# precice/fem-shell

Measured on AMD Instinct MI355X. Metric: elements assembled/s + CG iters/s, 4M-tri shell, 1/2/4/8 MI355X, higher is better.
Workload: dtype f64; 1 GPU; configs[3] flat panel 1414x1414 squares: 3998792 tri3, 12013350 dofs; parallelism=row-partition x1, rccl_ranks_seen=0, assembly_step=one femshell_assemble: launch + status round trip, warmup_step=one femshell_assemble + cg_iters CG iterations

## Files before the change

fem-shell_amd/binding.py:

```python
import ctypes as C
import os
import subprocess

import numpy as np

_HERE = os.path.dirname(os.path.abspath(__file__))
_CSRC = os.path.join(_HERE, "csrc")

REF_Y21 = 0x1
REF_DRILL_MAX = 0x2
REASSEMBLE_EACH_SOLVE = 0x4
REF_DEFAULT = REF_Y21 | REF_DRILL_MAX
REORDER_MORTON = 0x10
REORDER_RCM = 0x20

KERNEL_ASSEMBLE, KERNEL_SPMV, KERNEL_CG_UPDATE, KERNEL_CG_DIRECTION = 0, 1, 2, 3
KERNEL_LUMPED_MASS, KERNEL_MASS_SHIFT, KERNEL_NEWMARK_RHS, KERNEL_NEWMARK_UPDATE = 4, 5, 6, 7
KERNEL_SPMM, KERNEL_GRAM, KERNEL_BLOCK_COMBINE = 8, 9, 10
KERNEL_ELEMENT_PRODUCT = 11
KERNEL_ELEMENT_RESULTANTS = 12
KERNEL_ELEMENT_LOADS = 13
KERNEL_GEOMETRIC_PRODUCT = 14

SYMBOLS = [
    "femshell_create", "femshell_destroy", "femshell_last_error", "femshell_set_mesh",
    "femshell_set_dirichlet", "femshell_set_loads", "femshell_assemble", "femshell_assemble_async", "femshell_solve",
    "femshell_get_solution", "femshell_residual_history", "femshell_element_matrices",
    "femshell_nnz_blocks", "femshell_export_bsr", "femshell_spmv", "femshell_row_begin",
    "femshell_row_end", "femshell_comm_unique_id", "femshell_comm_init", "femshell_time_kernel",
    "femshell_sync", "femshell_pc_defaults", "femshell_set_preconditioner", "femshell_amg_levels", "femshell_amg_level",
    "femshell_amg_export", "femshell_residual", "femshell_comm_ranks", "femshell_amg_setup_stats", "femshell_amg_dense_stats", "femshell_amg_partition_info", "femshell_assembly_kernel",
    "femshell_amg_cycle_bytes", "femshell_comm_selftest", "femshell_comm_counters", "femshell_owned_nodes", "femshell_comm_bytes", "femshell_set_initial_guess",
    "femshell_amg_patch_info", "femshell_amg_symbolic_info", "femshell_pc_apply", "femshell_set_sections",
    "femshell_set_density", "femshell_lumped_mass", "femshell_dynamics_defaults", "femshell_dynamics_begin", "femshell_dynamics_step",
    "femshell_dynamics_accept", "femshell_dynamics_state", "femshell_dynamics_energy", "femshell_dynamics_end",
    "femshell_modal_defaults", "femshell_modes", "femshell_spmm", "femshell_modal_gram",
    "femshell_set_prescribed", "femshell_reactions", "femshell_element_product", "femshell_element_resultants",
    "femshell_set_element_loads", "femshell_element_load_vector",
    "femshell_geometric_product", "femshell_buckling_defaults", "femshell_buckling",
    "femshell_pool_stats", "femshell_amg_device_dense_inverse", "femshell_amg_dense_apply",
    "femshell_amg_device_block_jacobi", "femshell_block_jacobi_export", "femshell_block_jacobi_apply",
]


class FemShellError(RuntimeError):
    def __init__(self, code, msg):
# ... 123 lines not shown
    L.femshell_sync.argtypes = [vp]
    L.femshell_pc_defaults.argtypes = [C.c_int32, C.POINTER(PcOptions)]
    L.femshell_set_preconditioner.argtypes = [vp, C.POINTER(PcOptions)]
    L.femshell_amg_levels.argtypes = [vp]
    L.femshell_amg_levels.restype = C.c_int32
    L.femshell_amg_level.argtypes = [vp, C.c_int32, C.POINTER(AmgLevelInfo)]
    L.femshell_amg_export.argtypes = [vp, C.c_int32, C.c_int32, C.c_void_p]
    L.femshell_amg_export.restype = C.c_int64
    L.femshell_amg_setup_stats.argtypes = [vp, dp]
    L.femshell_amg_dense_stats.argtypes = [vp, dp]
    L.femshell_amg_patch_info.argtypes = [vp, dp]
    L.femshell_amg_symbolic_info.argtypes = [vp, ip]
    L.femshell_pc_apply.argtypes = [vp, dp, dp]
    L.femshell_amg_partition_info.argtypes = [vp, dp]
    L.femshell_assembly_kernel.argtypes = [vp]
    L.femshell_comm_selftest.argtypes = [vp, dp]
    L.femshell_comm_counters.argtypes = [vp, C.POINTER(C.c_int64), C.c_int32]
    L.femshell_comm_bytes.argtypes = [vp, C.POINTER(C.c_int64), C.c_int32]
    L.femshell_amg_cycle_bytes.argtypes = [vp, dp, C.c_int32]
    L.femshell_amg_cycle_bytes.restype = C.c_int32
    L.femshell_set_density.argtypes = [vp, C.c_double, C.c_int32, dp]
    L.femshell_lumped_mass.argtypes = [vp, dp]
    L.femshell_dynamics_defaults.argtypes = [C.POINTER(DynamicsOptions)]
    L.femshell_dynamics_begin.argtypes = [vp, C.POINTER(DynamicsOptions), dp, dp]
    L.femshell_dynamics_step.argtypes = [vp, C.c_double, C.c_int32, C.POINTER(SolveInfo)]
    L.femshell_dynamics_accept.argtypes = [vp]
    L.femshell_dynamics_state.argtypes = [vp, C.c_int32, dp, dp, dp]
    L.femshell_dynamics_energy.argtypes = [vp, C.c_int32, dp]
    L.femshell_dynamics_end.argtypes = [vp]
    L.femshell_modal_defaults.argtypes = [C.POINTER(ModalOptions)]
# ... 388 lines not shown
        _check(self._L.femshell_amg_setup_stats(self._h, _d(out)))
        return {"prolongator_ms": out[0], "ap_ms": out[1], "restriction_ms": out[2], "galerkin_ms": out[3],
                "galerkin_useful_flops": out[4], "galerkin_mfma_flops_issued": out[5], "galerkin_on_matrix_cores": bool(out[6])}

    def amg_symbolic_info(self):
        out = np.zeros(3, dtype=np.int32)
        _check(self._L.femshell_amg_symbolic_info(self._h, _i(out)))
        return {"in_hbm": int(out[0]), "host_after_overflow": int(out[1]), "host_by_rule": int(out[2])}

    def assembly_kernel(self):
        k = self._L.femshell_assembly_kernel(self._h)
        if k < 0:
            _check(k)
        return "k_assemble_pipe" if k == 1 else "k_assemble"

    def amg_dense_stats(self):
        out = np.zeros(6)
        _check(self._L.femshell_amg_dense_stats(self._h, _d(out)))
        return {"n": int(out[0]), "ms": out[1], "mfma_flops_issued": out[2], "useful_flops": out[3], "dropped_directions": int(out[4]),
                "bytes": out[5]}

    def amg_device_dense_inverse(self, rowptr, colidx, vals, single_precision=False):
        rowptr = np.ascontiguousarray(rowptr, dtype=np.int32)
        colidx = np.ascontiguousarray(colidx, dtype=np.int32)
        vals = np.ascontiguousarray(vals, dtype=np.float64)
        n = 6 * (len(rowptr) - 1)
        inv, out = np.zeros((n, n)), np.zeros(6)
        _check(self._L.femshell_amg_device_dense_inverse(self._h, len(rowptr) - 1, _i(rowptr), _i(colidx), _d(vals),
                                                         1 if single_precision else 0, _d(inv), _d(out)))
        return inv, {"n": int(out[0]), "ms": out[1], "mfma_flops_issued": out[2], "useful_flops": out[3],
# ... 370 lines not shown
```

fem-shell_amd/csrc/api.cpp:

```cpp
#include "api_internal.hpp"
#include "reorder.hpp"

#include <algorithm>
#include <atomic>
#include <chrono>
#include <cmath>
#include <cstdio>
#include <cstdlib>
#include <cstring>

using namespace femshell;

namespace femshell {

namespace {
thread_local std::string g_err;

struct ProductBuffers {
    DevBuf<double> x, y;
    std::vector<double> stage;
    int upload(femshell_ctx *c, NodeOrder order, const double *hx)
    {
        const size_t ld = (size_t)c->plan.n_local_nodes() * 6;
        FS_HIP(y.alloc((size_t)c->plan.n_pad * 6));
// ... 614 lines not shown
    if (!c || !out) return set_err(FEMSHELL_ERR_INVALID, "femshell_comm_bytes: null argument");
    out[0] = c->comm.halo_bytes_sent;
    out[1] = c->comm.collective_bytes;
    if (clear) c->comm.halo_bytes_sent = c->comm.collective_bytes = 0;
    return c->comm.active() ? 1 : 0;
}

int femshell_comm_selftest(femshell_ctx *c, double out_us[3])
{
    if (!c || !out_us) return set_err(FEMSHELL_ERR_INVALID, "femshell_comm_selftest: null argument");
    for (int i = 0; i < 3; i++) out_us[i] = c->comm_selftest_done ? c->comm_selftest_us[i] : -1.0;
    return c->comm_selftest_done ? 1 : 0;
}

int32_t femshell_comm_ranks(femshell_ctx *c) { return c ? comm_count(c->comm) : 0; }

static int set_mesh_on_this_rank(femshell_ctx *c, int32_t n_nodes, const double *xyz, int32_t n_tri, const int32_t *tri,
                                 int32_t n_quad, const int32_t *quad)
{
    int rc = FEMSHELL_OK;
    TraceRange trace("femshell_set_mesh (plan + upload)");
    static const bool verbose = plan_verbose();
    double t_part = wall_s();
    auto part_done = [&](const char *what) {
        const double t = wall_s();
        if (verbose) fprintf(stderr, "[femshell set_mesh] %-40s %.3f s\n", what, t - t_part);
        t_part = t;
    };
    if (!all_finite(xyz, 3ll * n_nodes)) return set_err(FEMSHELL_ERR_MESH, "femshell_set_mesh: non-finite coordinate");
    std::string e;
// ... 103 lines not shown
    c->dm.cols = c->cols.p;
    c->dm.pair_ptr = c->pair_ptr.p;
    c->dm.slice_elem_ptr = c->slice_elem_ptr.p;
    c->dm.slice_elem_nodes = reinterpret_cast<const int4 *>(c->slice_elem_nodes.p);
    c->dm.max_slice_elems = p.max_slice_elems;
    c->dm.max_slice_width = p.max_slice_width;
    c->dm.item_ptr = c->item_ptr.p;
    c->dm.slice_desc = reinterpret_cast<const int4 *>(c->slice_desc.p);
    c->dm.items = reinterpret_cast<const uint4 *>(c->items.p);
    FS_HIP(c->item_flags.alloc(p.pipe ? 0 : p.items.size()));
    c->dm.item_flags = c->item_flags.p;
    c->dm.max_stage_rows = p.max_stage_rows;
    c->dm.pipe = p.pipe ? 1 : 0;
    c->pipe_without_sections = p.pipe;
    c->dm.slice_elem_ptr_last = (int32_t)(p.slice_elem_nodes.size() / 4);
    {
        const size_t lds = assemble_lds_layout(c->dm, p.max_slice_elems, p.max_stage_rows, p.n_lquad() > 0);
        if (p.max_slice_width > 64) return set_err(FEMSHELL_ERR_UNSUPPORTED, "femshell_set_mesh: a node has more than 63 neighbours");
        if (lds > 160 * 1024)
            return set_err(FEMSHELL_ERR_UNSUPPORTED, "femshell_set_mesh: a 32-node slice touches too many elements for the LDS staging");
    }
    c->dm.vals = c->vals.p;
    c->dm.symmetric = p.symmetric ? 1 : 0;
    c->dm.diag_upper = (p.symmetric && knob_flag("FEMSHELL_DIAG_UPPER", true)) ? 1 : 0;
    c->dm.max_in_width = p.max_in_width;
    c->dm.in_width = c->in_width.p;
    c->dm.in_base = c->in_base.p;
    c->dm.in_slots = c->in_slots.p;
    c->dm.in_rows = c->in_rows.p;
    const bool local_products = p.symmetric && p.max_loc > 0 && knob_flag("FEMSHELL_SPMV_LOCAL", true);
// ... 123 lines not shown
static int upload_item_layout(femshell_ctx *c, bool sections)
{
    const Plan &p = c->plan;
    hipStream_t st = c->stream;
    FS_HIP(hipStreamSynchronize(st));
    FS_HIP(c->item_ptr.upload(p.item_ptr, st));
    FS_HIP(c->slice_desc.upload(p.slice_desc, st));
    FS_HIP(c->items.upload(p.items, st));
    FS_HIP(c->item_flags.alloc(p.pipe ? 0 : p.items.size()));
    c->dm.item_ptr = c->item_ptr.p;
    c->dm.slice_desc = reinterpret_cast<const int4 *>(c->slice_desc.p);
    c->dm.items = reinterpret_cast<const uint4 *>(c->items.p);
    c->dm.item_flags = c->item_flags.p;
    c->dm.max_stage_rows = p.max_stage_rows;
    c->dm.pipe = p.pipe ? 1 : 0;
    (void)assemble_lds_layout(c->dm, p.max_slice_elems, p.max_stage_rows, p.n_lquad() > 0, sections);
    launch_item_flags(c->dm, (int64_t)p.items.size(), st);
    FS_HIP(hipGetLastError());
    FS_HIP(hipStreamSynchronize(st));
    return FEMSHELL_OK;
}

int femshell_set_sections(femshell_ctx *c, int32_t n_sections, const femshell_section *sections, const int32_t *tri_section,
                          const int32_t *quad_section)
{
    if (!c) return set_err(FEMSHELL_ERR_INVALID, "femshell_set_sections: null context");
    if (const int prc = finish_pending_assembly(c)) return prc;
    if (!c->have_mesh) return set_err(FEMSHELL_ERR_INVALID, "femshell_set_sections: call femshell_set_mesh first");
    if (c->dyn.active) return set_err(FEMSHELL_ERR_INVALID, "femshell_set_sections: not while dynamics is active (femshell_dynamics_end first)");
    if (n_sections < 0) return set_err(FEMSHELL_ERR_INVALID, "femshell_set_sections: n_sections < 0");
// ... 276 lines not shown
    if (!c) return set_err(FEMSHELL_ERR_INVALID, "femshell_amg_cycle_bytes: null context");
    if (!c->amg || !c->amg->valid) return set_err(FEMSHELL_ERR_INVALID, "femshell_amg_cycle_bytes: no multigrid hierarchy");
    std::vector<double> b;
    (void)amg_cycle_bytes(c, &b);
    for (int32_t l = 0; per_level != nullptr && l < cap && l < (int32_t)b.size(); l++) per_level[l] = b[(size_t)l];
    return (int32_t)b.size();
}

int femshell_assembly_kernel(femshell_ctx *c)
{
    if (!c) return set_err(FEMSHELL_ERR_INVALID, "femshell_assembly_kernel: null context");
    if (!c->have_mesh) return set_err(FEMSHELL_ERR_INVALID, "femshell_assembly_kernel: no mesh");
    return c->dm.pipe ? 1 : 0;
}

int femshell_amg_dense_stats(femshell_ctx *c, double out[6])
{
    if (!c || !out) return set_err(FEMSHELL_ERR_INVALID, "femshell_amg_dense_stats: null argument");
    if (!c->amg || !c->amg->valid) return set_err(FEMSHELL_ERR_INVALID, "femshell_amg_dense_stats: no multigrid hierarchy");
    const AmgDenseStats &S = c->amg->dense;
    out[0] = (double)S.n;
    out[1] = S.ms;
    out[2] = S.mfma_flops;
    out[3] = S.useful_flops;
    out[4] = (double)S.dropped;
    out[5] = S.bytes;
    return FEMSHELL_OK;
}

int femshell_amg_device_dense_inverse(femshell_ctx *c, int32_t n_nodes, const int32_t *rowptr, const int32_t *colidx, const double *vals,
// ... 453 lines not shown
```

fem-shell_amd/csrc/assemble_kernel.hpp:

```cpp
#pragma once

#include "device_common.hpp"
#include "kernels.hpp"
#include "plan.hpp"

namespace femshell {

__device__ __forceinline__ void lds_barrier()
{
    asm volatile("s_waitcnt lgkmcnt(0)\n\ts_barrier" ::: "memory");
}

template <int kWavesPerSimd, int kAblate = 0, bool kHasQuads = false, bool kSections = false>
__global__ __launch_bounds__(256, kWavesPerSimd) void k_assemble(DeviceMatrix m, MatConst mc, DeviceSections ds)
{
    extern __shared__ double lds[];
    double *lds_rec = lds + m.lds_rec_off;
    double *lds_stage = lds + m.lds_stage_off;
    constexpr int kRec = kHasQuads ? kRecDoublesQuad : kRecDoubles;
    const int tid = threadIdx.x;
    constexpr int kThreads = 256;
    const int etid = kThreads - 1 - tid;

    unsigned long long tacc[8] = {0, 0, 0, 0, 0, 0, 0, 0}, tprev = 0;
// ... 334 lines not shown
    return __hiloint2double(hi2, lo2);
}

__device__ __forceinline__ double unspecified_double()
{
    double x;
    asm volatile("" : "=v"(x));
    return x;
}

constexpr int kPipeConsumers = 192;
constexpr int kPipeFlagShift = 9;
static_assert(kFlagDiagBit + 1 + kPipeFlagShift <= 32 && kFlagValenceMask >= (uint32_t)(kItemPairs * 255), "the constraint word must fit item.w and hold the count of 255 chunks");
constexpr int kPipeRecPasses = 3;

template <int kAblate = 0, bool kHasQuads = false, bool kSections = false>
__global__ __launch_bounds__(256, 2) void k_assemble_pipe(DeviceMatrix m, MatConst mc, DeviceSections ds)
{
    constexpr bool kSecConsume = kSections && !(kAblate & 256), kSecProduce = kSections && !(kAblate & 512);
    extern __shared__ double lds[];
    __shared__ int simd_of_wave[4];
    constexpr int kRec = kHasQuads ? kRecDoublesQuad : (kSections ? RecLeanSec::doubles : RecLean::doubles);
    constexpr int kCoords = kHasQuads ? 12 : 9;
    const int tid = threadIdx.x, lane = tid & 63, wave = tid >> 6;
    int vwave;
    {
        unsigned hw;
        asm volatile("s_getreg_b32 %0, hwreg(HW_REG_HW_ID)" : "=s"(hw));
        const int simd = (int)((hw >> 4) & 3u);
        if (lane == 0) simd_of_wave[wave] = simd;
        __syncthreads();
// ... 12 lines not shown
            asm volatile("s_memtime %0\n\ts_waitcnt lgkmcnt(0)" : "=s"(tnow)::"memory");
            if (slot >= 0) tacc[slot] += tnow - tprev;
            tprev = tnow;
        }
    };
    stamp(-1);
    auto desc_a_of = [&](int s_) { return (s_ < w.last) ? m.slice_desc[2 * s_] : make_int4(0, 0, 0, 0); };
    auto desc_b_of = [&](int s_) { return (s_ < w.last) ? m.slice_desc[2 * s_ + 1] : make_int4(0, 0, 0, 0); };

    if (vwave == 3) {
        const int4 *enodes = m.slice_elem_nodes;
        const int32_t *esec = ds.slice_elem_section;
        const int n_entries = m.slice_elem_ptr_last;
        struct Range {
            int e0, ne;
        };
        auto passes_of = [&](int r0, const Range &a) { return (a.ne > r0) ? (a.ne - r0 + 63) >> 6 : 0; };
        auto stream_elem = [&](int r0, const Range &a, const Range &b, int slot) {
            const int last = max(passes_of(r0, a) - 1, 0);
            const int pi = (slot < kPipeRecPasses - 1) ? (slot < last ? slot : 0) : last;
            const int li = r0 + 64 * pi + lane, li2 = li - a.ne;
            int e = (li < a.ne) ? a.e0 + li : ((li2 < b.ne) ? b.e0 + li2 : a.e0 + max(a.ne - 1, 0));
            return min(max(e, 0), n_entries - 1);
        };
        auto carry_of = [&](int r0, const Range &a, const Range &b) {
            return min(max(r0 + 64 * passes_of(r0, a) - a.ne, 0), b.ne);
        };
        auto fetch_coords = [&](const int4 &c, double X[kCoords]) {
            const double *pa = m.xyz + 3 * (int64_t)c.x, *pb = m.xyz + 3 * (int64_t)c.y, *pc = m.xyz + 3 * (int64_t)c.z;
            X[0] = pa[0]; X[1] = pa[1]; X[2] = pa[2];
            X[3] = pb[0]; X[4] = pb[1]; X[5] = pb[2];
            X[6] = pc[0]; X[7] = pc[1]; X[8] = pc[2];
            if (kHasQuads) {
                const double *pd = m.xyz + 3 * (int64_t)(c.w >= 0 ? c.w : c.x);
                X[kCoords - 3] = pd[0]; X[kCoords - 2] = pd[1]; X[kCoords - 1] = pd[2];
            }
        };
        auto range_of = [&](const int4 &a) {
            Range r;
            r.e0 = __builtin_amdgcn_readfirstlane(a.x);
            r.ne = __builtin_amdgcn_readfirstlane(a.y);
            return r;
        };
        if (!(kAblate & 64)) __builtin_amdgcn_s_setprio(3);
        int s_build = w.s;
        Range ra = range_of(desc_a_of(s_build)), rb = range_of(desc_a_of(s_build + w.step)),
              rc = range_of(desc_a_of(s_build + 2 * w.step));
        int4 dvec = desc_a_of(s_build + 3 * w.step);
        int r0 = 0;
        int r0n = carry_of(r0, ra, rb);
        double X[kPipeRecPasses][kCoords];
        int4 ndn[kPipeRecPasses];
        bool is_quad[kPipeRecPasses];
        SecConst scx[kPipeRecPasses] = {};
        int secn[kPipeRecPasses] = {};
#pragma unroll
        for (int p = 0; p < kPipeRecPasses; p++) {
            const int4 c0 = enodes[stream_elem(r0, ra, rb, p)];
            fetch_coords(c0, X[p]);
            is_quad[p] = kHasQuads && c0.w >= 0;
            ndn[p] = enodes[stream_elem(r0n, rb, rc, p)];
            if (kSecProduce) {
                scx[p] = fetch_section(ds.table, esec[stream_elem(r0, ra, rb, p)]);
                secn[p] = esec[stream_elem(r0n, rb, rc, p)];
            }
// ... 27 lines not shown
#pragma unroll
                for (int q = 0; q < kRecDoubles; q++) rec[q] = 1.0 + 0.01 * q + Xp[q % 9] * 1e-9;
                ok = true;
            } else {
                ok = tri3_record(Xp, me, rec);
            }
#pragma unroll
            for (int q = 0; q < RecLean::doubles; q++) lean[q] = rec[lean_from_full(q)];
            if (kSections) {
#pragma unroll
                for (int q = RecLean::doubles; q < kRec; q++) lean[q] = 0.0;
                lean[RecLeanSec::nu] = ok ? me.nu : 0.0;
            }
            return ok;
        };
        auto produce = [&](double *buf) {
            if (held_at >= 0) write_lean(buf, held_at, held);
            held_at = -1;
            const int np = passes_of(r0, ra);
#pragma unroll
            for (int p = 0; p < kPipeRecPasses - 1; p++) {
                if (p < np - 1) {
                    double lean[kRec];
                    const bool ok = record_of(X[p], is_quad[p], scx[p], lean);
                    const int li = r0 + 64 * p + lane;
                    if (!ok) report_status(m.status, ra.e0 + li + 1);
                    write_lean(buf, li, lean);
                }
                fetch_coords(ndn[p], X[p]);
                is_quad[p] = kHasQuads && ndn[p].w >= 0;
                if (kSecProduce) scx[p] = fetch_section(ds.table, secn[p]);
// ... 11 lines not shown
            } else {
#pragma unroll
                for (int q = 0; q < kRec; q++) held[q] = 0.0;
            }
            fetch_coords(ndn[kPipeRecPasses - 1], X[kPipeRecPasses - 1]);
            is_quad[kPipeRecPasses - 1] = kHasQuads && ndn[kPipeRecPasses - 1].w >= 0;
            if (kSecProduce) scx[kPipeRecPasses - 1] = fetch_section(ds.table, secn[kPipeRecPasses - 1]);
            const Range rd = range_of(dvec);
            const int r0nn = carry_of(r0n, rb, rc);
            r0 = r0n;
            r0n = r0nn;
            ra = rb;
            rb = rc;
            rc = rd;
            s_build += w.step;
#pragma unroll
            for (int p = 0; p < kPipeRecPasses; p++) ndn[p] = enodes[stream_elem(r0n, rb, rc, p)];
            if (kSecProduce) {
#pragma unroll
                for (int p = 0; p < kPipeRecPasses; p++) secn[p] = esec[stream_elem(r0n, rb, rc, p)];
            }
            dvec = desc_a_of(s_build + 3 * w.step);
        };
        produce(lds);
        stamp(0);
        lds_barrier();
        stamp(1);
        for (int j = 0; j < n_iter; j++) {
            if (j + 1 < n_iter) produce(lds + (size_t)((j + 1) & 1) * m.lds_rec_off);
            stamp(0);
            lds_barrier();
            stamp(1);
        }
    } else {
        const int vtid = vwave * 64 + lane;
        if ((kAblate & 1024) && vwave == 1) __builtin_amdgcn_s_setprio(3);
        if ((kAblate & 2048) && vwave == 0) __builtin_amdgcn_s_setprio(1);
        struct Desc {
            int e0, ne, i0, ni;
            int64_t base;
        };
        auto decode = [&](const int4 &a, const int4 &b) {
            Desc d;
            d.e0 = __builtin_amdgcn_readfirstlane(a.x);
            d.ne = __builtin_amdgcn_readfirstlane(a.y);
            d.i0 = __builtin_amdgcn_readfirstlane(a.z);
            d.ni = __builtin_amdgcn_readfirstlane(a.w);
            d.base = (int64_t)(((uint64_t)(uint32_t)__builtin_amdgcn_readfirstlane(b.y) << 32) |
                               (uint32_t)__builtin_amdgcn_readfirstlane(b.x));
            return d;
        };
        Desc d0 = decode(desc_a_of(w.s), desc_b_of(w.s)), d1 = decode(desc_a_of(w.s + w.step), desc_b_of(w.s + w.step));
        int4 dva = desc_a_of(w.s + 2 * w.step), dvb = desc_b_of(w.s + 2 * w.step);
        double rhs_pre = 0.0;
        uint32_t rhs_mask = 0u;
        auto fetch_rhs = [&](int s_) {
            if (m.rhs_F != nullptr && s_ < w.last) {
                rhs_pre = m.rhs_loads[(int64_t)s_ * kSliceRows + vtid];
                rhs_mask = m.dmask[s_ * kSliceNodes + vtid / 6];
            }
        };
        fetch_rhs(w.s);
        uint4 item_pre = make_uint4(0xffffu, 0, 0, 0);
        if (vtid < d0.ni) item_pre = m.items[d0.i0 + vtid];
        lds_barrier();
        stamp(1);
        for (int j = 0; j < n_iter; j++, w.next()) {
            const int s = w.s;
            const double *lds_rec = lds + (size_t)(j & 1) * m.lds_rec_off;
            const int64_t base = d0.base;
            const int i0 = d0.i0, ni = d0.ni;
            uint4 item = item_pre;
            asm volatile("" : "+v"(item.x), "+v"(item.y), "+v"(item.z), "+v"(item.w));
            const Desc d2 = decode(dva, dvb);
            if (m.rhs_F != nullptr) {
                const bool fixed = (rhs_mask >> (vtid % 6)) & 1u;
                m.rhs_F[(int64_t)s * kSliceRows + vtid] = (fixed || s * kSliceNodes + vtid / 6 >= m.n_own) ? 0.0 : rhs_pre;
            }
            stamp(5);
            dva = desc_a_of(s + 3 * w.step);
            dvb = desc_b_of(s + 3 * w.step);
            fetch_rhs(s + w.step);
            uint4 item_next = make_uint4(0xffffu, 0, 0, 0);
            if (vtid < d1.ni) item_next = m.items[d1.i0 + vtid];
            stamp(6);
            double2 *out = reinterpret_cast<double2 *>(m.vals + base * 36);
            for (int r0 = 0; r0 < ni; r0 += kPipeConsumers) {
                const int it = r0 + vtid;
                const bool live = it < ni;
                if (r0 > 0) {
                    item = make_uint4(0xffffu, 0, 0, 0);
                    if (live) item = m.items[i0 + it];
                    asm volatile("" : "+v"(item.x), "+v"(item.y), "+v"(item.z), "+v"(item.w));
                }
                const int slot_in_slice = (int)(item.x & 0xffffu), chunk = (int)((item.x >> 16) & 0xffu),
                          nchunks = (int)(item.x >> 24);
                const int cnt = (int)((item.z >> 16) & 0xffu);
                const bool general = (item.z >> 31) != 0u;
                const int wave_chunks = __builtin_amdgcn_readfirstlane((int)(item.w & 0xffu));
                const bool wave_sym = !kHasQuads && __builtin_amdgcn_readfirstlane((int)((item.w >> 8) & 1u)) != 0;
                const bool sym_item = !kHasQuads && slot_in_slice < kSliceNodes && !general;
                auto add_diag = [&](uint32_t pr, double acc[21]) {
                    const double *rec = lds_rec + pipe_rec_offset((int)(pr >> 4), kRec);
                    if (kSecConsume) tri3_diag_add_rec<RecLean>(rec, (int)(pr & 3u), rec_material_lean(rec, mc.flags), acc);
                    else tri3_diag_add_rec<RecLean>(rec, (int)(pr & 3u), mc, acc);
// ... 149 lines not shown
```

fem-shell_amd/csrc/kernels.hip:

```cpp
#include "kernels.hpp"
#include "plan.hpp"
#include "device_common.hpp"

#include <type_traits>
#include "assemble_kernel.hpp"

#include <cstdlib>

namespace femshell {

static_assert(kSliceNodes == 32 && kSliceRows == 192, "kernels assume 32-node slices");

static int assemble_grid(const DeviceMatrix &m)
{
    static const int cap = grid_cap(knob_text("FEMSHELL_ASM_GRID"), 2048);
    const int g = 8 * ((m.n_slices + 7) / 8);
    return g < cap ? g : cap;
}

int slice_grid(const DeviceMatrix &m)
{
    static const int cap = grid_cap(knob_text("FEMSHELL_SLICE_GRID"), 65536);
    const int g = 8 * ((m.n_slices + 7) / 8);
    return g < cap ? g : cap;
}

#ifndef FEMSHELL_SECTIONS_LAB
#define FEMSHELL_SECTIONS_LAB 0
#endif
constexpr int kSectionsLab = FEMSHELL_SECTIONS_LAB;

bool launch_assemble(const DeviceMatrix &m, const MatConst &mc, hipStream_t st, const DeviceSections *sections)
{
    const size_t lds = (size_t)m.lds_bytes;
    const DeviceSections ds = sections ? *sections : DeviceSections();
    const int g = assemble_grid(m);
    auto launch = [&](auto kernel) {
        if (lds > 64 * 1024)
            (void)hipFuncSetAttribute(reinterpret_cast<const void *>(kernel), hipFuncAttributeMaxDynamicSharedMemorySize, (int)lds);
        hipLaunchKernelGGL(kernel, dim3(g), dim3(256), lds, st, m, mc, ds);
    };
    if (sections && (!ds.table || !ds.slice_elem_section)) return false;
    if (m.pipe) {
        static const int pipe_cap = [] {
            int dev = 0, cus = 0;
            if (hipGetDevice(&dev) != hipSuccess || hipDeviceGetAttribute(&cus, hipDeviceAttributeMultiprocessorCount, dev) != hipSuccess || cus <= 0)
                cus = 256;
            return grid_cap(knob_text("FEMSHELL_ASM_PIPE_GRID"), 8 * ((2 * cus + 7) / 8));
        }();
        const int gp = g < pipe_cap ? g : pipe_cap;
        auto launch_pipe = [&](auto kernel) {
            if (lds > 64 * 1024)
                (void)hipFuncSetAttribute(reinterpret_cast<const void *>(kernel), hipFuncAttributeMaxDynamicSharedMemorySize, (int)lds);
            hipLaunchKernelGGL(kernel, dim3(gp), dim3(256), lds, st, m, mc, ds);
        };
        if (sections) {
            if (m.n_lquad > 0) launch_pipe(k_assemble_pipe<0, true, true>);
            else launch_pipe(k_assemble_pipe<kSectionsLab, false, true>);
        } else if (m.n_lquad > 0) {
            launch_pipe(k_assemble_pipe<0, true>);
        } else {
            launch_pipe(k_assemble_pipe<0, false>);
        }
        return true;
    }
    if (sections) {
        if (m.n_lquad > 0) launch(k_assemble<2, 0, true, true>);
        else launch(k_assemble<2, 0, false, true>);
        return true;
    }
    if (m.n_lquad > 0) launch(k_assemble<2, 0, true>);
    else launch(k_assemble<2, 0, false>);
    return true;
}

__global__ __launch_bounds__(256) void k_item_flags(DeviceMatrix m)
{
    for (int s = blockIdx.x; s < m.n_slices; s += gridDim.x) {
// ... 193 lines not shown
```

fem-shell_amd/csrc/kernels.hpp:

```cpp
#pragma once

#include <hip/hip_runtime.h>
#include <stdint.h>

#include "shell_element.hpp"

namespace femshell {

constexpr int32_t kStatusDirect = 0x40000000;
constexpr uint32_t kFlagValenceMask = 1023u;
constexpr int kFlagDiagBit = 22;

struct DeviceMatrix {
    int32_t n_own = 0, n_pad = 0, n_ghost = 0, n_slices = 0;
    int32_t n_ltri = 0, n_lquad = 0;
    const double *xyz = nullptr;
    const int32_t *tri = nullptr;
    const int32_t *quad = nullptr;
    const int32_t *slice_width = nullptr;
    const int64_t *slice_base = nullptr;
    const int32_t *cols = nullptr;
    const int32_t *pair_ptr = nullptr;
    const int32_t *slice_elem_ptr = nullptr;
    const int4 *slice_desc = nullptr;
    const int4 *slice_elem_nodes = nullptr;
    int32_t max_slice_elems = 0;
    int32_t max_slice_width = 0;
    const int32_t *item_ptr = nullptr;
    const uint4 *items = nullptr;
    uint32_t *item_flags = nullptr;
    int32_t max_stage_rows = 0;
    int32_t lds_bytes = 0;
    int32_t lds_rec_off = 0, lds_stage_off = 0;
    int32_t pipe = 0;
    int32_t slice_elem_ptr_last = 0;
    const uint8_t *dmask = nullptr;
    double *vals = nullptr;
    const float *vals32 = nullptr;
    int32_t vec32 = 0;
    const double *rhs_loads = nullptr;
    double *rhs_F = nullptr;
    int32_t symmetric = 0;
    int32_t diag_upper = 0;
    int32_t max_in_width = 0;
    const int32_t *in_width = nullptr;
    const int64_t *in_base = nullptr;
    const int32_t *in_slots = nullptr;
    const int32_t *in_rows = nullptr;
    const int32_t *gat_slots = nullptr;
// ... 1 lines not shown
    const uint8_t *loc_list = nullptr;
    int32_t max_loc = 0;
    double *tbuf = nullptr;
    double *minv = nullptr;
    const float *minv32 = nullptr;
    unsigned long long *stamps = nullptr;
    int32_t *status = nullptr;
};

#ifndef FEMSHELL_PIPE_REC_PAD
#define FEMSHELL_PIPE_REC_PAD 0
#endif
constexpr int kPipeRecPad = FEMSHELL_PIPE_REC_PAD;
__host__ __device__ constexpr int pipe_rec_offset(int i, int rec_doubles) { return i * rec_doubles + kPipeRecPad * (i >> 4); }

inline size_t assemble_lds_layout(DeviceMatrix &m, int32_t max_slice_elems, int32_t max_stage_rows, bool has_quads,
                                  bool sections = false)
{
    if (m.pipe) {
        m.lds_rec_off = pipe_rec_offset(max_slice_elems, has_quads ? kRecDoublesQuad : (sections ? RecLeanSec::doubles : RecLean::doubles));
        m.lds_stage_off = 0;
        m.lds_bytes = (int32_t)(2 * (size_t)m.lds_rec_off * sizeof(double));
        return (size_t)m.lds_bytes;
    }
    const int rec = has_quads ? kRecDoublesQuad : kRecDoubles;
    m.lds_rec_off = 0;
    m.lds_stage_off = max_slice_elems * rec;
    m.lds_bytes = (int32_t)(((size_t)max_slice_elems * rec + (size_t)max_stage_rows * 36) * sizeof(double));
    return (size_t)m.lds_bytes;
}
struct CgScalars {
    double rz;
    double alpha;
    double beta;
    double rr;
    double bb;
    double tol2;
// ... 23 lines not shown

enum CgPhase : int {
    CG_PHASE_NONE = 0, CG_PHASE_INIT = 1, CG_PHASE_ALPHA = 2, CG_PHASE_BETA = 3, CG_PHASE_RESTART = 4,
    CG_PHASE_FUSED_INIT = 5, CG_PHASE_FUSED_STEP = 6,
    CG_PHASE_FLEX_INIT = 7,
    CG_PHASE_FLEX_RZ0 = 8,
    CG_PHASE_FLEX_CONV = 9,
    CG_PHASE_FLEX_BETA = 10,
    CG_PHASE_FLEX_RESTART = 11,
    CG_PHASE_FLEX_WARM = 12
};

int slice_grid(const DeviceMatrix &m);

bool launch_assemble(const DeviceMatrix &m, const MatConst &mc, hipStream_t st, const DeviceSections *sections = nullptr);
void launch_rhs(const DeviceMatrix &m, const double *loads , double *F, hipStream_t st);
void launch_item_flags(const DeviceMatrix &m, int64_t n_items, hipStream_t st);
void launch_block_jacobi(const DeviceMatrix &m, hipStream_t st);
void launch_status_flags(const int32_t *status, double *agree, hipStream_t st);
void launch_element_matrices(const DeviceMatrix &m, const MatConst &mc, int32_t first, int32_t count,
                             double *Ke_out, hipStream_t st, const DeviceSections *sections = nullptr);

void launch_element_product(const DeviceMatrix &m, const MatConst &mc, const DeviceSections *sections, const double *x, const double *xp,
                            const double *sub, double *y, bool rhs, hipStream_t st);

void launch_element_resultants(const DeviceMatrix &m, const MatConst &mc, const DeviceSections *sections, const double *sec_t, const double *u,
                               const double *up, double *out, hipStream_t st);

void launch_element_loads(const DeviceMatrix &m, const int32_t *slice_elem_local, const double *elem_load, const double *base, double *out,
                          hipStream_t st);
// ... 57 lines not shown
```

include/femshell.h:

```cpp
#ifndef FEMSHELL_H
#define FEMSHELL_H

#include <stdint.h>

#ifdef __cplusplus
extern "C" {
#endif

#define FEMSHELL_VERSION 2

typedef enum femshell_status {
    FEMSHELL_OK = 0,
    FEMSHELL_ERR_INVALID = -1,
    FEMSHELL_ERR_NO_DEVICE = -2,
    FEMSHELL_ERR_HIP = -3,
    FEMSHELL_ERR_MESH = -4,
    FEMSHELL_ERR_BREAKDOWN = -5,
    FEMSHELL_ERR_COMM = -6,
    FEMSHELL_ERR_UNSUPPORTED = -7
} femshell_status;

#define FEMSHELL_REF_Y21        0x1u
#define FEMSHELL_REF_DRILL_MAX  0x2u
#define FEMSHELL_REASSEMBLE_EACH_SOLVE 0x4u
// ... 93 lines not shown
int femshell_amg_setup_stats(femshell_ctx *ctx, double out[7]);
int femshell_amg_symbolic_info(femshell_ctx *ctx, int32_t out[3]);
int femshell_amg_dense_stats(femshell_ctx *ctx, double out[6]);
int femshell_amg_device_dense_inverse(femshell_ctx *ctx, int32_t n_nodes, const int32_t *rowptr, const int32_t *colidx,
                                      const double *vals, int32_t single_precision, double *inv_out, double stats_out[6]);
int femshell_amg_dense_apply(femshell_ctx *ctx, int32_t n, int32_t n_pad6, const double *inv, int32_t as_float, const double *b,
                             double *y);
int femshell_amg_device_block_jacobi(femshell_ctx *ctx, int32_t n_nodes, const int32_t *rowptr, const int32_t *colidx,
                                     const double *vals, int32_t symmetric_storage, double *inv_out, int32_t *status_out);
int femshell_block_jacobi_export(femshell_ctx *ctx, int32_t level, int32_t single_precision, double *out);
int femshell_block_jacobi_apply(femshell_ctx *ctx, int32_t level, int32_t path, const double *r, double *z);
int femshell_pool_stats(double out[6]);
int femshell_amg_partition_info(femshell_ctx *ctx, double out[6]);
int32_t femshell_amg_cycle_bytes(femshell_ctx *ctx, double *per_level, int32_t cap);
int femshell_assembly_kernel(femshell_ctx *ctx);

int femshell_solve(femshell_ctx *ctx, double rtol, int32_t max_it, double *u_out,
                   femshell_solve_info *info);
int femshell_get_solution(femshell_ctx *ctx, double *u_out);
int femshell_reactions(femshell_ctx *ctx, const double *u , double *r6_out );
int femshell_element_resultants(femshell_ctx *ctx, const double *u , double *out );
int femshell_set_initial_guess(femshell_ctx *ctx, const double *u0);
int32_t femshell_residual_history(femshell_ctx *ctx, double *hist, int32_t cap);

int femshell_set_density(femshell_ctx *ctx, double rho, int32_t n_sections, const double *section_rho);
int femshell_lumped_mass(femshell_ctx *ctx, double *m6_out);

typedef struct femshell_dynamics_options { double dt, beta, gamma, alpha; } femshell_dynamics_options;
int femshell_dynamics_defaults(femshell_dynamics_options *out);
int femshell_dynamics_begin(femshell_ctx *ctx, const femshell_dynamics_options *opt, const double *u0, const double *v0);
// ... 83 lines not shown
```

Baseline: 6.998 billion elements/s.

## Feed consumer slice headers and items through LDS from producer wave in pipe assembly

```diff
diff --git a/fem-shell_amd/binding.py b/fem-shell_amd/binding.py
--- a/fem-shell_amd/binding.py
+++ b/fem-shell_amd/binding.py
@@ -29,7 +29,7 @@
     "femshell_nnz_blocks", "femshell_export_bsr", "femshell_spmv", "femshell_row_begin",
     "femshell_row_end", "femshell_comm_unique_id", "femshell_comm_init", "femshell_time_kernel",
     "femshell_sync", "femshell_pc_defaults", "femshell_set_preconditioner", "femshell_amg_levels", "femshell_amg_level",
-    "femshell_amg_export", "femshell_residual", "femshell_comm_ranks", "femshell_amg_setup_stats", "femshell_amg_dense_stats", "femshell_amg_partition_info", "femshell_assembly_kernel",
+    "femshell_amg_export", "femshell_residual", "femshell_comm_ranks", "femshell_amg_setup_stats", "femshell_amg_dense_stats", "femshell_amg_partition_info", "femshell_assembly_kernel", "femshell_assembly_feed_info",
     "femshell_amg_cycle_bytes", "femshell_comm_selftest", "femshell_comm_counters", "femshell_owned_nodes", "femshell_comm_bytes", "femshell_set_initial_guess",
     "femshell_amg_patch_info", "femshell_amg_symbolic_info", "femshell_pc_apply", "femshell_set_sections",
     "femshell_set_density", "femshell_lumped_mass", "femshell_dynamics_defaults", "femshell_dynamics_begin", "femshell_dynamics_step",
@@ -183,6 +183,7 @@
     L.femshell_pc_apply.argtypes = [vp, dp, dp]
     L.femshell_amg_partition_info.argtypes = [vp, dp]
     L.femshell_assembly_kernel.argtypes = [vp]
+    L.femshell_assembly_feed_info.argtypes = [vp, C.POINTER(C.c_int64)]
     L.femshell_comm_selftest.argtypes = [vp, dp]
     L.femshell_comm_counters.argtypes = [vp, C.POINTER(C.c_int64), C.c_int32]
     L.femshell_comm_bytes.argtypes = [vp, C.POINTER(C.c_int64), C.c_int32]
@@ -601,6 +602,11 @@
             _check(k)
         return "k_assemble_pipe" if k == 1 else "k_assemble"
 
+    def assembly_feed_info(self):
+        out = np.zeros(4, dtype=np.int64)
+        _check(self._L.femshell_assembly_feed_info(self._h, out.ctypes.data_as(C.POINTER(C.c_int64))))
+        return {"fed": bool(out[0]), "lds_bytes": int(out[1]), "blocks_per_cu": int(out[2]), "max_slice_items": int(out[3])}
+
     def amg_dense_stats(self):
         out = np.zeros(6)
         _check(self._L.femshell_amg_dense_stats(self._h, _d(out)))
diff --git a/fem-shell_amd/csrc/api.cpp b/fem-shell_amd/csrc/api.cpp
--- a/fem-shell_amd/csrc/api.cpp
+++ b/fem-shell_amd/csrc/api.cpp
@@ -652,6 +652,13 @@
 }
 
 int32_t femshell_comm_ranks(femshell_ctx *c) { return c ? comm_count(c->comm) : 0; }
+
+static int32_t max_slice_items(const Plan &p)
+{
+    int32_t most = 0;
+    for (size_t s = 0; s + 1 < p.item_ptr.size(); s++) most = std::max(most, p.item_ptr[s + 1] - p.item_ptr[s]);
+    return most;
+}
 
 static int set_mesh_on_this_rank(femshell_ctx *c, int32_t n_nodes, const double *xyz, int32_t n_tri, const int32_t *tri,
                                  int32_t n_quad, const int32_t *quad)
@@ -785,6 +792,8 @@
     c->dm.pipe = p.pipe ? 1 : 0;
     c->pipe_without_sections = p.pipe;
     c->dm.slice_elem_ptr_last = (int32_t)(p.slice_elem_nodes.size() / 4);
+    c->dm.feed_wanted = knob_flag("FEMSHELL_ASM_FEED", true) ? 1 : 0;
+    c->dm.max_slice_items = max_slice_items(p);
     {
         const size_t lds = assemble_lds_layout(c->dm, p.max_slice_elems, p.max_stage_rows, p.n_lquad() > 0);
         if (p.max_slice_width > 64) return set_err(FEMSHELL_ERR_UNSUPPORTED, "femshell_set_mesh: a node has more than 63 neighbours");
@@ -938,6 +947,7 @@
     c->dm.item_flags = c->item_flags.p;
     c->dm.max_stage_rows = p.max_stage_rows;
     c->dm.pipe = p.pipe ? 1 : 0;
+    c->dm.max_slice_items = max_slice_items(p);
     (void)assemble_lds_layout(c->dm, p.max_slice_elems, p.max_stage_rows, p.n_lquad() > 0, sections);
     launch_item_flags(c->dm, (int64_t)p.items.size(), st);
     FS_HIP(hipGetLastError());
@@ -1244,6 +1254,19 @@
     return c->dm.pipe ? 1 : 0;
 }
 
+int femshell_assembly_feed_info(femshell_ctx *c, int64_t out[4])
+{
+    if (!c || !out) return set_err(FEMSHELL_ERR_INVALID, "femshell_assembly_feed_info: null argument");
+    if (!c->have_mesh) return set_err(FEMSHELL_ERR_INVALID, "femshell_assembly_feed_info: no mesh");
+    const int rc = select_device(c);
+    if (rc) return rc;
+    out[0] = c->dm.pipe_fed;
+    out[1] = c->dm.lds_bytes;
+    out[2] = assemble_blocks_per_cu(c->dm, c->sections_or_null() != nullptr);
+    out[3] = c->dm.max_slice_items;
+    return FEMSHELL_OK;
+}
+
 int femshell_amg_dense_stats(femshell_ctx *c, double out[6])
 {
     if (!c || !out) return set_err(FEMSHELL_ERR_INVALID, "femshell_amg_dense_stats: null argument");
diff --git a/fem-shell_amd/csrc/assemble_kernel.hpp b/fem-shell_amd/csrc/assemble_kernel.hpp
--- a/fem-shell_amd/csrc/assemble_kernel.hpp
+++ b/fem-shell_amd/csrc/assemble_kernel.hpp
@@ -372,7 +372,7 @@
 static_assert(kFlagDiagBit + 1 + kPipeFlagShift <= 32 && kFlagValenceMask >= (uint32_t)(kItemPairs * 255), "the constraint word must fit item.w and hold the count of 255 chunks");
 constexpr int kPipeRecPasses = 3;
 
-template <int kAblate = 0, bool kHasQuads = false, bool kSections = false>
+template <int kAblate = 0, bool kHasQuads = false, bool kSections = false, bool kFed = false>
 __global__ __launch_bounds__(256, 2) void k_assemble_pipe(DeviceMatrix m, MatConst mc, DeviceSections ds)
 {
     constexpr bool kSecConsume = kSections && !(kAblate & 256), kSecProduce = kSections && !(kAblate & 512);
@@ -415,6 +415,7 @@
         const int n_entries = m.slice_elem_ptr_last;
         struct Range {
             int e0, ne;
+            int i0, ni;
         };
         auto passes_of = [&](int r0, const Range &a) { return (a.ne > r0) ? (a.ne - r0 + 63) >> 6 : 0; };
         auto stream_elem = [&](int r0, const Range &a, const Range &b, int slot) {
@@ -441,6 +442,8 @@
             Range r;
             r.e0 = __builtin_amdgcn_readfirstlane(a.x);
             r.ne = __builtin_amdgcn_readfirstlane(a.y);
+            r.i0 = kFed ? __builtin_amdgcn_readfirstlane(a.z) : 0;
+            r.ni = kFed ? __builtin_amdgcn_readfirstlane(a.w) : 0;
             return r;
         };
         if (!(kAblate & 64)) __builtin_amdgcn_s_setprio(3);
@@ -450,6 +453,41 @@
         int4 dvec = desc_a_of(s_build + 3 * w.step);
         int r0 = 0;
         int r0n = carry_of(r0, ra, rb);
+        constexpr bool kFeedAhead = !kSections;
+        uint4 hitem[3] = {make_uint4(0xffffu, 0, 0, 0), make_uint4(0xffffu, 0, 0, 0), make_uint4(0xffffu, 0, 0, 0)};
+        int4 hdesc = make_int4(0, 0, 0, 0);
+        double hload[3] = {0.0, 0.0, 0.0};
+        uint32_t hmask = 0u;
+        auto fetch_header = [&](int s_, const Range &a) {
+            const int sc = min(s_, m.n_slices - 1);
+            const int4 dw = m.slice_desc[2 * sc + (lane & 1)];
+            hdesc = (s_ < w.last) ? dw : make_int4(0, 0, 0, 0);
+#pragma unroll
+            for (int k = 0; k < 3; k++) {
+                const int v = lane + 64 * k;
+                const uint4 it = m.items[max(a.i0 + min(v, a.ni - 1), 0)];
+                hitem[k] = (v < a.ni) ? it : make_uint4(0xffffu, 0, 0, 0);
+            }
+            const double *lp = (m.rhs_F != nullptr) ? m.rhs_loads + ((int64_t)sc * kSliceRows + 3 * lane) : m.xyz;
+#pragma unroll
+            for (int k = 0; k < 3; k++) hload[k] = lp[k];
+            hmask = m.dmask[sc * kSliceNodes + (lane >> 1)];
+        };
+        auto write_header = [&](int jj, int s_) {
+            uint4 *hdr = reinterpret_cast<uint4 *>(lds + 2 * (size_t)m.lds_rec_off) + (size_t)(jj & 1) * kPipeHeaderWords;
+            if (lane < 2) hdr[lane] = make_uint4((uint32_t)hdesc.x, (uint32_t)hdesc.y, (uint32_t)hdesc.z, (uint32_t)hdesc.w);
+#pragma unroll
+            for (int k = 0; k < 3; k++) hdr[2 + lane + 64 * k] = hitem[k];
+            if (m.rhs_F != nullptr) {
+                const bool beyond = s_ * kSliceNodes + (lane >> 1) >= m.n_own;
+#pragma unroll
+                for (int k = 0; k < 3; k++) {
+                    const bool fixed = (hmask >> (3 * (lane & 1) + k)) & 1u;
+                    m.rhs_F[(int64_t)s_ * kSliceRows + 3 * lane + k] = (fixed || beyond) ? 0.0 : hload[k];
+                }
+            }
+        };
+        if (kFed) fetch_header(s_build, ra);
         double X[kPipeRecPasses][kCoords];
         int4 ndn[kPipeRecPasses];
         bool is_quad[kPipeRecPasses];
@@ -507,7 +545,11 @@
             }
             return ok;
         };
-        auto produce = [&](double *buf) {
+        auto produce = [&](double *buf, int jj) {
+            if (kFed) {
+                write_header(jj, s_build);
+                if (kFeedAhead) fetch_header(s_build + w.step, rb);
+            }
             if (held_at >= 0) write_lean(buf, held_at, held);
             held_at = -1;
             const int np = passes_of(r0, ra);
@@ -549,6 +591,7 @@
             rb = rc;
             rc = rd;
             s_build += w.step;
+            if (kFed && !kFeedAhead) fetch_header(s_build, ra);
 #pragma unroll
             for (int p = 0; p < kPipeRecPasses; p++) ndn[p] = enodes[stream_elem(r0n, rb, rc, p)];
             if (kSecProduce) {
@@ -557,12 +600,12 @@
             }
             dvec = desc_a_of(s_build + 3 * w.step);
         };
-        produce(lds);
+        produce(lds, 0);
         stamp(0);
         lds_barrier();
         stamp(1);
         for (int j = 0; j < n_iter; j++) {
-            if (j + 1 < n_iter) produce(lds + (size_t)((j + 1) & 1) * m.lds_rec_off);
+            if (j + 1 < n_iter) produce(lds + (size_t)((j + 1) & 1) * m.lds_rec_off, j + 1);
             stamp(0);
             lds_barrier();
             stamp(1);
@@ -585,8 +628,14 @@
                                (uint32_t)__builtin_amdgcn_readfirstlane(b.x));
             return d;
         };
-        Desc d0 = decode(desc_a_of(w.s), desc_b_of(w.s)), d1 = decode(desc_a_of(w.s + w.step), desc_b_of(w.s + w.step));
-        int4 dva = desc_a_of(w.s + 2 * w.step), dvb = desc_b_of(w.s + 2 * w.step);
+        Desc d0 = {0, 0, 0, 0, 0}, d1 = d0;
+        int4 dva = make_int4(0, 0, 0, 0), dvb = dva;
+        if (!kFed) {
+            d0 = decode(desc_a_of(w.s), desc_b_of(w.s));
+            d1 = decode(desc_a_of(w.s + w.step), desc_b_of(w.s + w.step));
+            dva = desc_a_of(w.s + 2 * w.step);
+            dvb = desc_b_of(w.s + 2 * w.step);
+        }
         double rhs_pre = 0.0;
         uint32_t rhs_mask = 0u;
         auto fetch_rhs = [&](int s_) {
@@ -595,35 +644,46 @@
                 rhs_mask = m.dmask[s_ * kSliceNodes + vtid / 6];
             }
         };
-        fetch_rhs(w.s);
+        if (!kFed) fetch_rhs(w.s);
         uint4 item_pre = make_uint4(0xffffu, 0, 0, 0);
-        if (vtid < d0.ni) item_pre = m.items[d0.i0 + vtid];
+        if (!kFed && vtid < d0.ni) item_pre = m.items[d0.i0 + vtid];
         lds_barrier();
         stamp(1);
         for (int j = 0; j < n_iter; j++, w.next()) {
             const int s = w.s;
             const double *lds_rec = lds + (size_t)(j & 1) * m.lds_rec_off;
+            if (kFed) {
+                const uint4 *hdr = reinterpret_cast<const uint4 *>(lds + 2 * (size_t)m.lds_rec_off) + (size_t)(j & 1) * kPipeHeaderWords;
+                const uint4 ha = hdr[0], hb = hdr[1];
+                item_pre = hdr[2 + vtid];
+                d0 = decode(make_int4((int)ha.x, (int)ha.y, (int)ha.z, (int)ha.w), make_int4((int)hb.x, (int)hb.y, (int)hb.z, (int)hb.w));
+            }
             const int64_t base = d0.base;
             const int i0 = d0.i0, ni = d0.ni;
             uint4 item = item_pre;
             asm volatile("" : "+v"(item.x), "+v"(item.y), "+v"(item.z), "+v"(item.w));
-            const Desc d2 = decode(dva, dvb);
-            if (m.rhs_F != nullptr) {
-                const bool fixed = (rhs_mask >> (vtid % 6)) & 1u;
-                m.rhs_F[(int64_t)s * kSliceRows + vtid] = (fixed || s * kSliceNodes + vtid / 6 >= m.n_own) ? 0.0 : rhs_pre;
+            Desc d2 = d1;
+            if (!kFed) {
+                d2 = decode(dva, dvb);
+                if (m.rhs_F != nullptr) {
+                    const bool fixed = (rhs_mask >> (vtid % 6)) & 1u;
+                    m.rhs_F[(int64_t)s * kSliceRows + vtid] = (fixed || s * kSliceNodes + vtid / 6 >= m.n_own) ? 0.0 : rhs_pre;
+                }
             }
             stamp(5);
-            dva = desc_a_of(s + 3 * w.step);
-            dvb = desc_b_of(s + 3 * w.step);
-            fetch_rhs(s + w.step);
             uint4 item_next = make_uint4(0xffffu, 0, 0, 0);
-            if (vtid < d1.ni) item_next = m.items[d1.i0 + vtid];
+            if (!kFed) {
+                dva = desc_a_of(s + 3 * w.step);
+                dvb = desc_b_of(s + 3 * w.step);
+                fetch_rhs(s + w.step);
+                if (vtid < d1.ni) item_next = m.items[d1.i0 + vtid];
+            }
             stamp(6);
             double2 *out = reinterpret_cast<double2 *>(m.vals + base * 36);
-            for (int r0 = 0; r0 < ni; r0 += kPipeConsumers) {
+            for (int r0 = 0; r0 < (kFed ? min(ni, 1) : ni); r0 += kPipeConsumers) {
                 const int it = r0 + vtid;
                 const bool live = it < ni;
-                if (r0 > 0) {
+                if (!kFed && r0 > 0) {
                     item = make_uint4(0xffffu, 0, 0, 0);
                     if (live) item = m.items[i0 + it];
                     asm volatile("" : "+v"(item.x), "+v"(item.y), "+v"(item.z), "+v"(item.w));
diff --git a/fem-shell_amd/csrc/kernels.hip b/fem-shell_amd/csrc/kernels.hip
--- a/fem-shell_amd/csrc/kernels.hip
+++ b/fem-shell_amd/csrc/kernels.hip
@@ -29,6 +29,42 @@
 #define FEMSHELL_SECTIONS_LAB 0
 #endif
 constexpr int kSectionsLab = FEMSHELL_SECTIONS_LAB;
+
+template <class F> static void with_pipe_kernel(const DeviceMatrix &m, bool sections, F &&f)
+{
+    const bool fed = m.pipe_fed != 0;
+    if (sections) {
+        if (m.n_lquad > 0) f(k_assemble_pipe<0, true, true>);
+        else fed ? f(k_assemble_pipe<kSectionsLab, false, true, true>) : f(k_assemble_pipe<kSectionsLab, false, true>);
+    } else if (m.n_lquad > 0) {
+        f(k_assemble_pipe<0, true>);
+    } else {
+        fed ? f(k_assemble_pipe<0, false, false, true>) : f(k_assemble_pipe<0, false>);
+    }
+}
+
+int assemble_blocks_per_cu(const DeviceMatrix &m, bool sections)
+{
+    int blocks = -1;
+    auto query = [&](auto kernel) {
+        if (m.lds_bytes > 64 * 1024)
+            (void)hipFuncSetAttribute(reinterpret_cast<const void *>(kernel), hipFuncAttributeMaxDynamicSharedMemorySize, m.lds_bytes);
+        if (hipOccupancyMaxActiveBlocksPerMultiprocessor(&blocks, reinterpret_cast<const void *>(kernel), 256, (size_t)m.lds_bytes) != hipSuccess) {
+            (void)hipGetLastError();
+            blocks = -1;
+        }
+    };
+    if (m.pipe) {
+        with_pipe_kernel(m, sections, query);
+    } else if (sections) {
+        if (m.n_lquad > 0) query(k_assemble<2, 0, true, true>);
+        else query(k_assemble<2, 0, false, true>);
+    } else {
+        if (m.n_lquad > 0) query(k_assemble<2, 0, true>);
+        else query(k_assemble<2, 0, false>);
+    }
+    return blocks;
+}
 
 bool launch_assemble(const DeviceMatrix &m, const MatConst &mc, hipStream_t st, const DeviceSections *sections)
 {
@@ -54,14 +90,7 @@
                 (void)hipFuncSetAttribute(reinterpret_cast<const void *>(kernel), hipFuncAttributeMaxDynamicSharedMemorySize, (int)lds);
             hipLaunchKernelGGL(kernel, dim3(gp), dim3(256), lds, st, m, mc, ds);
         };
-        if (sections) {
-            if (m.n_lquad > 0) launch_pipe(k_assemble_pipe<0, true, true>);
-            else launch_pipe(k_assemble_pipe<kSectionsLab, false, true>);
-        } else if (m.n_lquad > 0) {
-            launch_pipe(k_assemble_pipe<0, true>);
-        } else {
-            launch_pipe(k_assemble_pipe<0, false>);
-        }
+        with_pipe_kernel(m, sections != nullptr, launch_pipe);
         return true;
     }
     if (sections) {
diff --git a/fem-shell_amd/csrc/kernels.hpp b/fem-shell_amd/csrc/kernels.hpp
--- a/fem-shell_amd/csrc/kernels.hpp
+++ b/fem-shell_amd/csrc/kernels.hpp
@@ -33,6 +33,7 @@
     int32_t lds_bytes = 0;
     int32_t lds_rec_off = 0, lds_stage_off = 0;
     int32_t pipe = 0;
+    int32_t feed_wanted = 0, max_slice_items = 0, pipe_fed = 0;
     int32_t slice_elem_ptr_last = 0;
     const uint8_t *dmask = nullptr;
     double *vals = nullptr;
@@ -64,13 +65,26 @@
 constexpr int kPipeRecPad = FEMSHELL_PIPE_REC_PAD;
 __host__ __device__ constexpr int pipe_rec_offset(int i, int rec_doubles) { return i * rec_doubles + kPipeRecPad * (i >> 4); }
 
+constexpr int kPipeHeaderWords = 2 + 192;
+constexpr int kPipeHeaderBytes = 2 * kPipeHeaderWords * 16;
+constexpr int kPipeStaticLds = 16;
+constexpr int kLdsPerCu = 160 * 1024, kLdsGranule = 1280;
+constexpr bool kPipeFedBuilt[2][2] = {{true, true}, {false, false}};
+
 inline size_t assemble_lds_layout(DeviceMatrix &m, int32_t max_slice_elems, int32_t max_stage_rows, bool has_quads,
                                   bool sections = false)
 {
+    m.pipe_fed = 0;
     if (m.pipe) {
         m.lds_rec_off = pipe_rec_offset(max_slice_elems, has_quads ? kRecDoublesQuad : (sections ? RecLeanSec::doubles : RecLean::doubles));
         m.lds_stage_off = 0;
         m.lds_bytes = (int32_t)(2 * (size_t)m.lds_rec_off * sizeof(double));
+        const size_t fed_bytes = (size_t)m.lds_bytes + kPipeHeaderBytes;
+        const size_t fed_alloc = (fed_bytes + kPipeStaticLds + kLdsGranule - 1) / kLdsGranule * kLdsGranule;
+        if (m.feed_wanted && kPipeFedBuilt[has_quads][sections] && m.max_slice_items <= 192 && 2 * fed_alloc <= (size_t)kLdsPerCu) {
+            m.pipe_fed = 1;
+            m.lds_bytes = (int32_t)fed_bytes;
+        }
         return (size_t)m.lds_bytes;
     }
     const int rec = has_quads ? kRecDoublesQuad : kRecDoubles;
@@ -124,6 +138,7 @@
 int slice_grid(const DeviceMatrix &m);
 
 bool launch_assemble(const DeviceMatrix &m, const MatConst &mc, hipStream_t st, const DeviceSections *sections = nullptr);
+int assemble_blocks_per_cu(const DeviceMatrix &m, bool sections);
 void launch_rhs(const DeviceMatrix &m, const double *loads , double *F, hipStream_t st);
 void launch_item_flags(const DeviceMatrix &m, int64_t n_items, hipStream_t st);
 void launch_block_jacobi(const DeviceMatrix &m, hipStream_t st);
diff --git a/include/femshell.h b/include/femshell.h
--- a/include/femshell.h
+++ b/include/femshell.h
@@ -131,6 +131,7 @@
 int femshell_amg_partition_info(femshell_ctx *ctx, double out[6]);
 int32_t femshell_amg_cycle_bytes(femshell_ctx *ctx, double *per_level, int32_t cap);
 int femshell_assembly_kernel(femshell_ctx *ctx);
+int femshell_assembly_feed_info(femshell_ctx *ctx, int64_t out[4]);
 
 int femshell_solve(femshell_ctx *ctx, double rtol, int32_t max_it, double *u_out,
                    femshell_solve_info *info);
```

After: 7.059 billion elements/s (median of 6 runs). Within noise of the previous version (+0.9%).
